# althonos/pyfastani

Measured on AMD Instinct MI355X. Metric: genome-pair ANI/sec (5 Mb bacterial, 3 kb frags), higher is better.
Workload: dtype u32

## Files before the change

### include/fastani_hip.h

```cpp
#ifndef FASTANI_HIP_H
#define FASTANI_HIP_H

#include <stdint.h>

#ifdef __cplusplus
extern "C" {
#endif

#define FA_OK 0
#define FA_ERR_INVALID 1
#define FA_ERR_NO_DEVICE 2
#define FA_ERR_NOMEM 3
#define FA_ERR_UNSUPPORTED 4
#define FA_ERR_INTERNAL 5
#define FA_ERR_IO 6
#define FA_ERR_BUFFER 7

typedef struct fa_sketch fa_sketch;
typedef struct fa_mapper fa_mapper;
typedef struct fa_genomes fa_genomes;

typedef struct fa_params {
  int32_t kmer_size;
  int32_t window_size;
// ... 119 lines not shown

int fa_mapper_debug_mappings(fa_mapper *m, fa_mapping *out, int64_t cap, int64_t *n);
int fa_mapper_debug_l1(fa_mapper *m, int32_t *frag, int32_t *seq_id, int32_t *range_start, int32_t *range_end,
                       int64_t cap, int64_t *n);
int fa_mapper_debug_query_sketch(fa_mapper *m, int64_t fragment, uint32_t *hashes, int32_t cap, int32_t *sketch_size);
int fa_debug_sketch_sequence(const fa_params *params, const void *data, int64_t length, int char_width,
                             uint32_t *hash, int32_t *wpos, int64_t cap, int64_t *n);

int fa_debug_probe_occupancy(int lds_bytes, int *peak_alive);
int fa_mapper_debug_items(fa_mapper *m, void *out, int64_t bytes);
int fa_mapper_debug_links(fa_mapper *m, int32_t *prev, int32_t *fwd, int32_t *bwd, uint8_t *flags, int64_t cap, int64_t *n);
int fa_mapper_debug_locus_events(fa_mapper *m, uint32_t *events, int64_t cap, int64_t *n);
int fa_mapper_last_timings(fa_mapper *m, float *ms, int n);
int fa_mapper_debug_spec(fa_mapper *m, int64_t *out, int n);
int fa_mapper_set_stage_events(fa_mapper *m, int on);
int fa_mapper_stream(fa_mapper *m, void **stream);
int fa_bench_sketch_kernel(fa_mapper *m, fa_genomes *g, int repeat, float *ms_per_launch, uint64_t *bases,
                           uint64_t *minimizers);

#ifdef __cplusplus
}
#endif
#endif
```

### pyfastani_amd/_lib.py

```python
import ctypes as C
import os

_HERE = os.path.dirname(os.path.abspath(__file__))
LIB_PATH = os.path.join(_HERE, "lib", "libfastani_hip.so")

FA_OK, FA_ERR_INVALID, FA_ERR_NO_DEVICE, FA_ERR_NOMEM, FA_ERR_UNSUPPORTED, FA_ERR_INTERNAL, FA_ERR_IO, FA_ERR_BUFFER = range(8)


class Params(C.Structure):
    _fields_ = [
        ("kmer_size", C.c_int32),
        ("window_size", C.c_int32),
        ("fragment_length", C.c_int32),
        ("alphabet_size", C.c_int32),
        ("min_fraction", C.c_float),
        ("percentage_identity", C.c_float),
        ("p_value", C.c_double),
        ("reference_size", C.c_uint64),
    ]


class CgiRow(C.Structure):
    _fields_ = [
        ("query_id", C.c_int32),
# ... 88 lines not shown
    "fa_packed_append": (_i32, [_vp, _P(C.c_char_p), _i32]),
    "fa_packed_free": (None, [_vp]),
    "fa_packed_info": (_i32, [_vp, _P(_i32), _P(C.c_uint64), _P(_i64), _P(_i64)]),
    "fa_sketch_add_packed": (_i32, [_vp, _vp, _i32, _i32, _P(_i64), _P(_i64)]),
    "fa_genomes_reload_packed": (_i32, [_vp, _vp, _vp, _i32, _i32]),
    "fa_genomes_reload_fasta": (_i32, [_vp, _vp, _P(C.c_char_p), _i32]),
    "fa_sketch_add_genomes": (_i32, [_vp, _P(_vp), _P(_i64), _P(_i32), _i64, _i32, _i32, _P(_i32)]),
    "fa_sketch_add_fasta_many": (_i32, [_vp, _P(C.c_char_p), _i32, _P(_i64), _P(_i64)]),
    "fa_debug_probe_occupancy": (_i32, [_i32, _P(_i32)]),
    "fa_mapper_debug_items": (_i32, [_vp, _vp, _i64]),
    "fa_mapper_debug_locus_events": (_i32, [_vp, _vp, _i64, _vp]),
    "fa_mapper_debug_links": (_i32, [_vp, _vp, _vp, _vp, _vp, _i64, _vp]),
    "fa_mapper_last_timings": (_i32, [_vp, _P(_f32), _i32]),
    "fa_mapper_debug_spec": (_i32, [_vp, _P(_i64), _i32]),
    "fa_mapper_set_stage_events": (_i32, [_vp, _i32]),
    "fa_mapper_stream": (_i32, [_vp, _P(_vp)]),
    "fa_bench_sketch_kernel": (_i32, [_vp, _vp, _i32, _P(_f32), _P(_u64), _P(_u64)]),
}

if not os.path.exists(LIB_PATH):
    raise ImportError(
        f"{LIB_PATH} is missing: build it with `python -c 'import __graft_entry__ as g; g.build()'` "
        "(hipcc --offload-arch=gfx950). pyfastani_amd has no CPU fallback."
    )



os.environ.setdefault("GPU_MAX_HW_QUEUES", "8")
lib = C.CDLL(LIB_PATH)
for _name, (_res, _args) in SIGNATURES.items():
# ... 32 lines not shown
```

### pyfastani_amd/csrc/fa_engine.hip

```cpp
#include <cstring>

#include <rocprim/rocprim.hpp>

#include <algorithm>
#include <atomic>
#include <chrono>
#include <climits>
#include <cstdlib>
#include <cstring>
#include <memory>
#include <condition_variable>
#include <mutex>
#include <shared_mutex>
#include <string>
#include <utility>
#include <vector>
#include <cstddef>
#include <deque>

#include "fa_common.h"
#include "fa_fasta.h"
#include "fa_lease.h"
#include "fa_map.hip.h"
#include "fa_policy.h"
// ... 395 lines not shown
  DevBuf<int32_t> map_chunk_count;
  DevBuf<int64_t> map_chunk_off;
  DevBuf<fa_hit_mapping> maps_dev;
  const int32_t *lut_min_hits = nullptr, *lut_pass = nullptr;
  const float *lut_ident = nullptr;
  int64_t last_F = 0;
  uint32_t last_loci = 0;
  uint32_t loci_n = 1, loci_shift = 0;
  uint32_t last_region_count[LOCI_REGIONS] = {0};
  uint64_t last_items = 0;
  const fa_genomes *last_genomes = nullptr;
  float last_ms[MS_SLOTS] = {0};
  hipEvent_t ev[6] = {nullptr};
  int64_t pass_F = 0;
  Forms forms, last_forms;
  std::unique_ptr<fa_genomes> query_batch;
  PinnedBuf pin_image, pin_rows;
  ~Workspace() {
    for (auto &e : ev) if (e) (void)hipEventDestroy(e);
    if (stream) (void)hipStreamDestroy(stream);
    if (h_status) (void)hipHostFree(h_status);
  }
};

struct fa_mapper {
  fa_params P;
  int device = -1;
  hipStream_t stream = nullptr;
  std::mutex mtx;
  DevBuf<uint32_t> rec_hash, uniq_hash, uniq_off, pos_ridx;
// ... 8 lines not shown
  bool events_packed() const { return packed_geo && !env_set("FA_NO_PACKED_GEO"); }
  int64_t N = 0, U = 0;
  int32_t C = 0, G = 0, table_bits = 4, freq_threshold = INT_MAX, total_bins = 0;
  std::vector<uint64_t> lengths;
  std::vector<int32_t> seqs_by_file;
  int32_t cmw = 0, qcap = 1;
  StatTables stats;
  DevBuf<int32_t> d_min_hits, d_pass;
  DevBuf<float> d_ident;
  Spec spec;
  static constexpr int NWS = 4;
  Workspace ws[NWS];
  std::condition_variable ws_free;
  int last_ws = 0;
  bool stage_events = false;
  std::vector<DevBuf<int32_t>> retired_i32;
  std::vector<DevBuf<float>> retired_f32;

  IndexView view() const {
    IndexView v;
    v.rec_hash = rec_hash.p; v.rec_seq = rec_seq.p; v.rec_wpos = rec_wpos.p; v.rec_prev = rec_prev.p; v.rec_fwd = rec_fwd.p; v.rec_bwd = rec_bwd.p; v.rec_flags = rec_flags.p;
    v.rec_hg = packed_geo ? rec_hg.p : nullptr; v.rec_prev16 = packed_geo ? rec_prev16.p : nullptr; v.rec_gpos = rec_gpos.p; v.wrap_rec = wrap_rec.p; v.n_wraps = n_wraps; v.gpos_bits = gpos_bits;
    v.uniq_hash = uniq_hash.p; v.uniq_off = uniq_off.p; v.pos_ridx = pos_ridx.p; v.table = table.p;
    v.contig_rec = contig_rec.p; v.contig_genome = contig_genome.p; v.contig_bin = contig_bin.p; v.genome_bin = genome_bin.p;
    v.N = N; v.U = U; v.C = C; v.G = G; v.table_bits = table_bits; v.freq_threshold = freq_threshold; v.total_bins = total_bins;
    return v;
  }
};

__global__ void k_contig_bins(const int32_t *contig_rec, const int32_t *rec_wpos, int C, int bin_len, int32_t *nbins) {
// ... 373 lines not shown
    ea.chunk_count = w.map_chunk_count.p; ea.chunk_off = w.map_chunk_off.p;
    ea.maps = maps.dev + maps.base; ea.cap = maps.cap - maps.base; ea.total_maps = &w.status.p->total_maps;
    if (map_chunks) hipLaunchKernelGGL(k_map_count, dim3(map_chunks), dim3(256), 0, st, ea);
    hipLaunchKernelGGL(k_map_scan, dim3(1), dim3(1024), 0, st, ea);
    if (map_chunks) hipLaunchKernelGGL(k_map_write, dim3(map_chunks), dim3(256), 0, st, ea);
  }
  struct Part {
    const Spec &sp;
    const int64_t f0, f1, F;
    const int t0, ntiles;
    const int smax;
    const int64_t l_cap;
    L1Plan l1;
    bool scan_sorted = false;
    bool wide = false;
    LociRegions loci{nullptr, 1, 0};
    const int32_t *frag_order = nullptr;
    uint32_t order_len = 0;
    Part(QueryPass &q, Run &r)
        : sp(r.sp), f0(r.f0), f1(r.f1), F(r.f1 - r.f0), t0(q.g.frag_tile_lo[r.f0]),
          ntiles(q.g.frag_tile_lo[r.f1] - q.g.frag_tile_lo[r.f0]), smax(r.sp.smax),
          l_cap(std::max<int64_t>(r.sp.l_cap, (int64_t)std::min<uint32_t>(LOCI_REGIONS, ev_regions_for(r.f1 - r.f0)))) {}
  };

  void launch_part(Run &r) {
    Part p(*this, r);
    const Spec &sp = p.sp;
    const int64_t f0 = p.f0, F = p.F;
    w.last_F = 0; w.last_loci = 0;
    const int ntiles = p.ntiles;
// ... 12 lines not shown
    const int64_t l_cap = p.l_cap;
    {
      static const L1Knobs knobs{(int)env_num("FA_L1_PREFILTER", -1), (float)env_num("FA_L1_THIN_SMALL", -1.0), (float)env_num("FA_L1_THIN_MID", 0.05)};
      p.l1 = plan_l1(sp, m.N, knobs);
      static const bool dbg_l1 = env_set("FA_DEBUG_L1");
      if (dbg_l1) fprintf(stderr, "k_l1 classes: need=%u tiny=%.3f small=%.3f mid=%.3f prefilter=%d -> %d launch(es)\n", p.l1.need, sp.l1_tiny_share, sp.l1_small_share, sp.l1_mid_share, (int)p.l1.prefilter, p.l1.n);
    }
    w.l_frag.ensure((size_t)l_cap); w.l_seq.ensure((size_t)l_cap); w.l_start.ensure((size_t)l_cap); w.l_end.ensure((size_t)l_cap + 4);
    w.l_rfirst.ensure((size_t)l_cap); w.l_rlast.ensure((size_t)l_cap + 4); w.l_rpart.ensure((size_t)l_cap);
    w.l_group.ensure((size_t)l_cap); w.l_shared.ensure((size_t)l_cap); w.l_pos.ensure((size_t)l_cap);
    w.group_best.ensure((size_t)l_cap + 2);
    w.l_beg.ensure((size_t)l_cap); w.l_end0.ensure((size_t)l_cap); w.l_last.ensure((size_t)l_cap); w.l_ndrop.ensure((size_t)l_cap);
    w.l_nev.ensure((size_t)l_cap); w.l_ioff.ensure((size_t)l_cap); w.l_redo.ensure((size_t)l_cap + 4);
    static const int scan_order_knob = (int)env_num("FA_L2_SCAN_ORDER", -1);
    p.scan_sorted = scan_sorted(sp, scan_order_knob);
    w.scan_hist.ensure((size_t)2 * LOCI_REGIONS * SCAN_CLASSES);
    if (p.scan_sorted) w.scan_order.ensure((size_t)l_cap + 64);
    w.ovf_buf.ensure((size_t)sp.scratch_words + 4);
    p.loci.count = w.status.p->loci_region;
    p.loci.n = std::min<uint32_t>(LOCI_REGIONS, ev_regions_for(F));
    p.loci.shift = (uint32_t)floor_log2((int)std::max<int64_t>(1, l_cap / p.loci.n));
    w.loci_n = p.loci.n; w.loci_shift = p.loci.shift;
    p.wide = wide_events(smax);
    w.items.ensure(((size_t)sp.items_cap + 8) * (p.wide ? 4 : 2));
    w.forms = Forms();
    w.forms.n_l1 = p.l1.n;
    for (int c = 0; c < p.l1.n; c++) w.forms.l1_threads[c] = p.l1.c[c].nt;
    w.forms.prefilter = p.l1.prefilter; w.forms.scan_sorted = p.scan_sorted; w.forms.wide = p.wide; w.forms.redo = sp.redo;
    w.forms.smax = smax; w.forms.seed_slots = p.l1.seed_slots();

    launch_sketch_stage(r, p);
    prepare_order(p);
    launch_l1_stage(p);
    launch_l2_stage(r, p);
    launch_cgi_stage_and_hand_over(r, p);
  }

  void prepare_order(Part &p) {
    static const bool order_on = env_num("FA_FRAG_ORDER", 1) != 0;
    static const bool order_one = env_num("FA_FRAG_ORDER_ONE", 1) != 0;
    if (!frag_order_gate(order_on, order_one, NQ, p.F)) return;
    if (w.order_batch != g.serial || w.order_f0 != p.f0 || w.order_f1 != p.f1) {
      std::vector<int32_t> ord;
// ... 125 lines not shown
      a.items = w.items.p; a.items_cap = sp.items_cap; a.pinfo = d_pinfo; a.l_cap = (int32_t)l_cap;
      a.l_shared = w.l_shared.p; a.l_pos = w.l_pos.p; a.pass_lut = w.lut_pass; a.group_best = w.group_best.p;
      a.counters = d_counters; a.loci = p.loci; a.qcap = qcap; a.cmw = m.cmw;
      a.cnt_slots = smax + 1;
      a.rec_total = (unsigned long long *)&d_totals[TOT_RECORDS];
      a.ev_region = w.status.p->ev_region; a.rec_region = w.status.p->rec_region;
      a.n_regions = ev_regions_for(F);
      a.region_cap = (sp.items_cap / a.n_regions) & ~7ULL;
      a.l_redo = w.l_redo.p;
      a.redo_count = &d_counters[CNT_WIDE];
      const L2Lds lds(m.P, smax, wide);
      a.scan_class_div = p.scan_sorted ? lds.scan_class_div : 0;
      a.scan_hist = w.scan_hist.p; a.scan_cursor = w.scan_hist.p + LOCI_REGIONS * SCAN_CLASSES;
      a.scan_order = p.scan_sorted ? w.scan_order.p : nullptr;
      a.f_loci_lo = w.f_loci_lo.p; a.f_loci_n = w.f_loci_n.p;
      a.frag_order = p.frag_order;
      const uint32_t ev_grid = p.frag_order ? p.order_len : (uint32_t)F;
      if (p.frag_order) r.ordered = true;
      a.ev_stage = lds.ev_stage;
      const size_t ev_lds = lds.events;
      FA_REQUIRE(ev_lds <= 150 * 1024, FA_ERR_UNSUPPORTED, "query sketch too large for the LDS-staged event kernel");
      auto pick_lanes = [&](int bytes) {
        int ln = L2_THREADS;
        while (ln > 1 && lds.scan(ln, bytes) > 144 * 1024) ln >>= 1;
        FA_REQUIRE(lds.scan(ln, bytes) <= 160 * 1024, FA_ERR_UNSUPPORTED, "query sketch too large for the LDS-resident L2 state");
        return ln;
      };
      const int lanes8 = pick_lanes(1), lanes16 = pick_lanes(2);
      const size_t lds8 = lds.scan(lanes8, 1), lds16 = lds.scan(lanes16, 2);
      auto scan_grid = [&](int lanes) { return (unsigned)(p.loci.n * (uint32_t)ceil_div((int64_t)1 << p.loci.shift, lanes)); };
      auto launch = [&](auto ev_kernel, auto scan8, auto scan8_rt, auto scan16, auto scan16_rt) {
        launch_lds(ev_kernel, dim3(ev_grid), dim3(EV_THREADS), ev_lds, st, a);
        debug_sync(st, "l2 events");
        if (p.scan_sorted)
          hipLaunchKernelGGL(k_l2_order, dim3((unsigned)(p.loci.n * (uint32_t)ceil_div((int64_t)1 << p.loci.shift, 256))), dim3(256), 0, st, a);
        a.lanes = lanes8;
        launch_lds(lanes8 == L2_THREADS ? scan8 : scan8_rt, dim3(scan_grid(lanes8)), dim3(L2_THREADS), lds8, st, a);
        if (!sp.redo) return;
        a.lanes = lanes16;
        launch_lds(lanes16 == L2_THREADS ? scan16 : scan16_rt, dim3(scan_grid(lanes16)), dim3(L2_THREADS), lds16, st, a);
      };
      const bool pk = m.events_packed();
      if (wide) launch(pk ? k_l2_events<uint32_t, true> : k_l2_events<uint32_t, false>, k_l2_scan<uint32_t, uint8_t, 64>, k_l2_scan<uint32_t, uint8_t, 0>, k_l2_scan<uint32_t, uint16_t, 64>, k_l2_scan<uint32_t, uint16_t, 0>);
      else launch(pk ? k_l2_events<uint16_t, true> : k_l2_events<uint16_t, false>, k_l2_scan<uint16_t, uint8_t, 64>, k_l2_scan<uint16_t, uint8_t, 0>, k_l2_scan<uint16_t, uint16_t, 64>, k_l2_scan<uint16_t, uint16_t, 0>);
    }
    debug_sync(st, "l2 scan");
    if (m.stage_events) FA_HIP(hipEventRecord(w.ev[3], st));
  }

  void launch_cgi_stage_and_hand_over(Run &r, Part &p) {
    const Spec &sp = p.sp;
    const int64_t f0 = p.f0;
    const int64_t l_cap = p.l_cap;
    uint32_t *const d_counters = w.status.p->counters;
    if (npairs > 0) {
      CgiArgs a;
      a.stamp = &w.status.p->stamp[3];
      a.ix = ix; a.group_best = w.group_best.p; a.counters = d_counters; a.l_frag = w.l_frag.p; a.l_seq = w.l_seq.p;
      a.l_pos = w.l_pos.p; a.q_size = w.q_size.p; a.ident_lut = w.lut_ident;
// ... 49 lines not shown
      w.last_ms[MS_L2_EVENTS] += ev_ms;
    }
    const unsigned long long *stamp = h.stamp;
    for (int i = 0; i < 4; i++) w.last_ms[MS_STAGE + i] += (float)((double)(stamp[i + 1] - stamp[i]) * 1e-5);
    t_begin = std::min(t_begin, stamp[0]); t_end = std::max(t_end, stamp[4]);
    w.last_F = F;
    w.last_loci = (uint32_t)v.loci;
    for (uint32_t i = 0; i < LOCI_REGIONS; i++)
      w.last_region_count[i] = i < w.loci_n ? (uint32_t)std::min<uint64_t>(h.loci_region[i], 1ULL << w.loci_shift) : 0u;
    w.last_items = v.events;
    const uint32_t *c = h.counters;
    w.last_ms[MS_RECORDS] += (float)v.records;
    w.last_ms[MS_LOCI] += (float)v.loci;
    w.last_ms[MS_EVENTS] += (float)v.events;
    w.last_ms[MS_WIDE] += (float)c[CNT_WIDE];
    w.last_ms[MS_L1_SORTED] += (float)c[CNT_L1_SORTED]; w.last_ms[MS_L1_MERGED] += (float)c[CNT_L1_MERGED];
    w.last_ms[MS_L1_OFF_FAST] += (float)(c[CNT_MERGED] + c[CNT_OFF_FAST]);
    if (c[CNT_L1_SORTED] + c[CNT_L1_MERGED] > 0) {
      const double nf = (double)(c[CNT_L1_SORTED] + c[CNT_L1_MERGED]);
      fprintf(stderr, "[fa] k_l1 phases, shader-clock ticks per fragment (thread 0):");
      for (int i = 0; i < 8; i++) fprintf(stderr, " %.0f", (double)h.dbg[i] / nf);
      fprintf(stderr, "  (%u block-sorted, %u merged; one workgroup in 64 sampled; gave up on probes / blocks / counts: %llu %llu %llu; expansion: bitmaps+places %.0f, pairs+bitmaps %.0f, bits %.0f)\n",
              c[CNT_L1_SORTED], c[CNT_L1_MERGED], h.dbg[8], h.dbg[9], h.dbg[10], (double)h.dbg[11] / nf, (double)h.dbg[12] / nf, (double)h.dbg[13] / nf);
    }
    return true;
  }


  int64_t run() {
    w.last_F = 0; w.last_loci = 0; w.last_genomes = &g;
// ... 45 lines not shown
    *maps.count = maps.base + pass.nmaps;
    FA_REQUIRE(pass.nmaps <= maps.cap - maps.base, FA_ERR_INVALID, "mapping buffer too small");
    maps.base += pass.nmaps;
  }
  return nrows;
}

struct MapRequest { fa_hit_mapping *maps; int64_t cap; int64_t *n_maps; bool device; };

static int64_t run_query(fa_mapper &m, Workspace &w, const fa_genomes &g, int32_t first, int32_t count, fa_cgi_row *rows, int64_t cap, bool rows_device,
                         const MapRequest *want = nullptr) {
  require_device();
  FA_REQUIRE(first >= 0 && count >= 0 && first + count <= g.n_genomes, FA_ERR_INVALID, "genome range out of bounds");
  for (float &x : w.last_ms) x = 0;
  w.last_forms = Forms();
  fa_cgi_row *dst = rows;
  if (!rows_device) { w.rows_dev.ensure((size_t)std::max<int64_t>(cap, 1)); dst = w.rows_dev.p; }
  const bool one_pass = count > 0 && g.genome_frag_lo[first + count] - g.genome_frag_lo[first] <= pass_fragments();
  fa_cgi_row *host_rows = nullptr;
  if (!rows_device && one_pass && cap <= 65536) {
    w.pin_rows.ensure(std::max<size_t>((size_t)cap * sizeof(fa_cgi_row), 4096));
    FA_HIP(hipHostGetDevicePointer((void **)&host_rows, w.pin_rows.p, 0));
  }
  MapSink sink;
  if (want) {
    FA_REQUIRE(want->cap >= 0 && (want->maps || want->cap == 0) && want->n_maps, FA_ERR_INVALID, "mapping buffer missing");
    sink.on = true; sink.cap = want->cap; sink.dev = want->maps; sink.count = want->n_maps;
    if (!want->device) { w.maps_dev.ensure((size_t)std::max<int64_t>(want->cap, 1)); sink.dev = w.maps_dev.p; }
    *want->n_maps = 0;
  }
// ... 967 lines not shown
      for_each_locus_slice(w, [&](size_t first, size_t count) {
        const size_t c = (size_t)std::max<int64_t>(0, std::min<int64_t>((int64_t)count, cap - k));
        if (c) FA_HIP(hipMemcpyAsync(events + k, w.l_nev.p + first, c * 4, hipMemcpyDeviceToHost, w.stream));
        k += (int64_t)count;
      });
      FA_HIP(hipStreamSynchronize(w.stream));
    }
    *n = k;
  });
}
int fa_mapper_set_stage_events(fa_mapper *m, int on) {
  std::lock_guard<std::mutex> lock(m->mtx);
  m->stage_events = on != 0;
  return FA_OK;
}
int fa_mapper_last_timings(fa_mapper *m, float *ms, int n) {
  std::lock_guard<std::mutex> lock(m->mtx);
  for (int i = 0; i < n && i < MS_SLOTS; i++) ms[i] = m->ws[m->last_ws].last_ms[i];
  return FA_OK;
}
int fa_mapper_debug_spec(fa_mapper *m, int64_t *out, int n) {
  std::lock_guard<std::mutex> lock(m->mtx);
  const Spec &s = m->spec;
  const Forms &f = m->ws[m->last_ws].last_forms;
  auto ppm = [](float share) { return (int64_t)std::lround((double)share * 1e6); };
  const int64_t v[] = {s.init, s.smax, s.seed_slots, ppm(s.l1_small_share), ppm(s.l1_mid_share), ppm(s.l1_tiny_share),
                       s.l1_prefilter, s.l1_no_small, s.l2_loci_last, s.redo, s.part_frags, s.fuse_skip, s.fuse_penalty,
                       s.smax_misses, (int64_t)s.scratch_words, (int64_t)s.items_cap, s.l_cap,
                       f.n_l1, f.l1_threads[0], f.l1_threads[1], f.l1_threads[2], f.prefilter, f.scan_sorted, f.wide, f.fused,
                       f.ordered, f.redo, f.smax, f.seed_slots};
  for (int i = 0; i < n; i++) out[i] = i < (int)(sizeof(v) / sizeof(v[0])) ? v[i] : 0;
  return FA_OK;
}
int fa_mapper_stream(fa_mapper *m, void **stream) { *stream = (void *)m->stream; return FA_OK; }

int fa_bench_sketch_kernel(fa_mapper *m, fa_genomes *g, int repeat, float *ms_per_launch, uint64_t *bases, uint64_t *minimizers) {
  return guarded([&] {
    WorkspaceLease lease(*m);
    Workspace &w = *lease.w;
    require_device();
    int ntiles = (int)g->ntiles;
    FA_REQUIRE(ntiles > 0 && repeat > 0, FA_ERR_INVALID, "nothing to sketch");
    const Tile *tiles = g->tiles;
    DevBuf<Tile> retiled;
    const int tile_len = k1_tile_len(m->P.window_size);
// ... 53 lines not shown
```

### pyfastani_amd/csrc/fa_map.hip.h

```cpp
#pragma once

#include "fa_common.h"
#include "fa_policy.h"
#include "fa_sketch.hip.h"
#include "fa_sketch_fast.hip.h"

namespace fa {



constexpr int MAP_THREADS = 256;
constexpr uint32_t SEED_PAD = 0xFFFFFFFFu;

__device__ inline void block_bitonic_sort(uint32_t *a, uint32_t n32) {
  for (uint32_t size = 2; size <= n32; size <<= 1) {
    for (uint32_t stride = size >> 1; stride > 0; stride >>= 1) {
      __syncthreads();
      for (uint32_t t = threadIdx.x; t < n32 / 2; t += blockDim.x) {
        uint32_t lo = 2 * t - (t & (stride - 1));
        uint32_t hi = lo + stride;
        bool up = (lo & size) == 0;
        uint32_t x = a[lo], y = a[hi];
        if ((x > y) == up) { a[lo] = y; a[hi] = x; }
      }
// ... 1620 lines not shown
  int32_t cnt_slots;
  int32_t lanes;
  int32_t ev_stage;
  unsigned long long *rec_total;
  unsigned long long *ev_region, *rec_region;
  uint64_t region_cap;
  uint32_t n_regions;
  uint8_t *l_redo;
  uint32_t *redo_count;
  const uint32_t *f_loci_lo, *f_loci_n;
  const int32_t *frag_order;
  unsigned long long *stamp;
  uint32_t *scan_hist, *scan_cursor;
  uint32_t *scan_order;
  int32_t scan_class_div;
};

constexpr int L2_THREADS = 64;
constexpr int EV_THREADS = 256;
constexpr int SCAN_CLASSES = 32;
__device__ __forceinline__ uint32_t scan_class(uint32_t nev, int32_t div) {
  return (uint32_t)(SCAN_CLASSES - 1) - min((uint32_t)(SCAN_CLASSES - 1), nev / (uint32_t)div);
}

template <typename T> struct EvBits;
template <> struct EvBits<uint16_t> { static constexpr int RANK = EV_RANK16; };
template <> struct EvBits<uint32_t> { static constexpr int RANK = 24; };
constexpr int EV_DM = 0, EV_DW = 2, EV_DROP = 5, EV_SLOT = 6;
template <typename T> constexpr uint32_t ev_noeval() { return 1u << (8 * sizeof(T) - 1); }
template <typename T> constexpr uint32_t ev_slot_mask() { return ((1u << EvBits<T>::RANK) - 1u) << EV_SLOT; }
// ... 274 lines not shown
  int lbase, LNB, s;
  int rl, g, shared, best, beg, opt_s, opt_e;
  uint32_t overflow;

  static __device__ __forceinline__ uint32_t ld(int addr) { return (uint32_t)*(lds_ptr)(uintptr_t)(uint32_t)addr; }
  static __device__ __forceinline__ void sto(int addr, uint32_t v) { *(lds_ptr)(uintptr_t)(uint32_t)addr = (ST)v; }

  __device__ __forceinline__ void init(ST *st, int lane, int lanes, int sketch, int beg0) {
    lbase = (int)(uint32_t)(uintptr_t)(lds_ptr)st + lane * STB;
    LNB = (LNT ? LNT : lanes) * STB;
    s = sketch;
    rl = lbase; g = 0; shared = 0; best = -1; beg = opt_s = opt_e = beg0; overflow = 0;
  }
  static constexpr uint32_t EMPTY = 2u;
  __device__ __forceinline__ void clear() { for (int i = 0; i <= s + 1; i++) sto(i * LNB + lbase, EMPTY); }
  template <int SH> __device__ __forceinline__ int slot_addr(uint32_t word) const {
    if constexpr (LNT == 64) {
      const uint32_t row = (SH ? word >> SH : word) & ev_slot_mask<T>();
      if constexpr (BASE0) return (int)((STB == 1 ? row : row * STB) | (uint32_t)lbase);
      else return (int)(STB == 1 ? row : row * STB) + lbase;
    } else {
      return (int)__builtin_amdgcn_ubfe(word, SH + EV_SLOT, RB) * LNB + lbase;
    }
  }
  template <int SH> __device__ __forceinline__ void fill(uint32_t word) {
    const int dM = __builtin_amdgcn_sbfe(word, SH + EV_DM, 2), dW = __builtin_amdgcn_sbfe(word, SH + EV_DW, 2);
    const int addr = slot_addr<SH>(word);
    const uint32_t nv = (ld(addr) + (uint32_t)(dW << 1)) ^ ((uint32_t)dM & 1u);
    overflow |= nv;
    sto(addr, nv);
  }
  __device__ __forceinline__ void read_pivot() {
    int rstar = s, F = s, acc = 0, m_acc = 0;
    bool hit = false;
    for (int r = 0; r < s; r++) {
      const uint32_t v = ld((r + 1) * LNB + lbase);
      const int c = (int)(v >> 1) - 1, mt = (int)(v & 1u);
      const bool now = !hit && r + acc + c >= s;
      rstar = now ? r : rstar;
      F = now ? r + acc : F;
      shared = now ? m_acc : shared;
      hit = hit || now;
      acc += c; m_acc += mt;
    }
    F = hit ? F : s + acc;
    shared = hit ? shared : m_acc;
    g = F - s;
    rl = rstar * LNB + lbase;
    best = shared;
  }
  template <int SH> __device__ __forceinline__ void step(uint32_t word) {
    const int dM = __builtin_amdgcn_sbfe(word, SH + EV_DM, 2), dW = __builtin_amdgcn_sbfe(word, SH + EV_DW, 2);
    const int drp = (int)__builtin_amdgcn_ubfe(word, SH + EV_DROP, 1);
    const int addr = slot_addr<SH>(word);
    const int addrb = rl + drp * LNB;
    const uint32_t v = ld(addr), vb0 = ld(addrb);
    const uint32_t nv = (v + (uint32_t)(dW << 1)) ^ ((uint32_t)dM & 1u);
    overflow |= nv;
    sto(addr, nv);
    const bool below = addr <= rl;
    const int dWb = below ? dW : 0;
    shared += below ? dM : 0;
    g += dWb;
    const uint32_t vb = (addrb == addr) ? nv : vb0;
// ... 22 lines not shown
  if (threadIdx.x < SCAN_CLASSES) sh_cnt[threadIdx.x] = 0;
  __syncthreads();
  const uint32_t l = (r << a.loci.shift) + off;
  uint32_t c = 0, rank = 0;
  if (off < live) { c = scan_class(a.l_nev[l], a.scan_class_div); rank = atomicAdd(&sh_cnt[c], 1u); }
  __syncthreads();
  if (threadIdx.x < SCAN_CLASSES) {
    uint32_t before = 0;
    for (uint32_t q = 0; q < threadIdx.x; q++) before += a.scan_hist[r * SCAN_CLASSES + q];
    sh_at[threadIdx.x] = before + (sh_cnt[threadIdx.x] ? atomicAdd(&a.scan_cursor[r * SCAN_CLASSES + threadIdx.x], sh_cnt[threadIdx.x]) : 0u);
  }
  __syncthreads();
  if (off < live) a.scan_order[(r << a.loci.shift) + min(sh_at[c] + rank, (1u << a.loci.shift) - 1u)] = l;
}

template <typename T, typename ST, int LNT>
__global__ __launch_bounds__(L2_THREADS) void k_l2_scan(L2Args a) {
  extern __shared__ __align__(16) unsigned char lds[];
  constexpr bool REDO = sizeof(ST) > 1;
  const int LN = LNT ? LNT : a.lanes;
  ST *st = (ST *)lds;
  const int lane = threadIdx.x;
  if (lane >= LN) return;
  const uint32_t region = blockIdx.x & (a.loci.n - 1u), off = (blockIdx.x / a.loci.n) * (uint32_t)LN + (uint32_t)lane;
  if (a.counters[CNT_LOCI_OVF] || off >= (1u << a.loci.shift) || off >= a.loci.count[region]) return;
  if (a.scan_order && a.pinfo[PI_FLAGS]) return;
  const uint32_t l = a.scan_order ? a.scan_order[(region << a.loci.shift) + off] : (region << a.loci.shift) + off;
  if (REDO) { if (!a.l_redo[l]) return; }
  else a.l_redo[l] = 0;
  const int s = a.q_size[a.l_frag[l]];
  if (s + 1 > a.cnt_slots) return;
  const int beg0 = a.l_beg[l];
  const uint32_t nev = a.l_nev[l];
  constexpr int PER = 16 / sizeof(T);
  const uint4 *ev = (const uint4 *)((const T *)a.items + a.l_ioff[l]);
  Slide<T, ST, LNT, true> sl;
  sl.init(st, lane, LN, s, beg0);
  sl.clear();
  if (sl.lbase != lane * (int)sizeof(ST)) __builtin_trap();

  const uint32_t ngroups = nev / PER;
  const uint32_t fill_groups = min(ngroups, (uint32_t)((((a.l_end0[l] - beg0) + 7) & ~7) / PER));
  auto word_of = [](const uint4 &g, int q) __attribute__((always_inline)) {
    constexpr int WPE = (int)sizeof(T);
    return (q * WPE / 4 == 0) ? g.x : (q * WPE / 4 == 1) ? g.y : (q * WPE / 4 == 2) ? g.z : g.w;
  };
  uint4 cur = ngroups ? ev[0] : make_uint4(0, 0, 0, 0);
  for (uint32_t g = 0; g < fill_groups; g++) {
    const uint4 nxt = (g + 1 < ngroups) ? ev[g + 1] : make_uint4(0, 0, 0, 0);
#pragma unroll
    for (int q = 0; q < PER; q++) {
      if (sizeof(T) == 2 && (q & 1)) sl.template fill<16>(word_of(cur, q)); else sl.template fill<0>(word_of(cur, q));
    }
    cur = nxt;
  }
  sl.read_pivot();
  if (!fill_groups) sl.best = -1;
  for (uint32_t g = fill_groups; g < ngroups; g++) {
    const uint4 nxt = (g + 1 < ngroups) ? ev[g + 1] : make_uint4(0, 0, 0, 0);
#pragma unroll
    for (int q = 0; q < PER; q++) {
      if (sizeof(T) == 2 && (q & 1)) sl.template step<16>(word_of(cur, q)); else sl.template step<0>(word_of(cur, q));
    }
    cur = nxt;
  }
  if (sl.overflow >> Slide<T, ST, LNT, true>::SBITS) {
    if (!REDO) { a.l_redo[l] = 1; atomicAdd(a.redo_count, 1u); return; }
  }
  a.l_shared[l] = sl.best < 0 ? 0 : sl.best;
  a.l_pos[l] = (a.ix.rec_wpos[sl.opt_s] + a.ix.rec_wpos[sl.opt_e]) / 2;
  if (sl.best >= a.pass_lut[s]) {
    unsigned long long key = ((unsigned long long)(uint32_t)sl.best << 32) | (unsigned long long)(0xFFFFFFFFu - l);
    atomicMax(&a.group_best[a.l_group[l]], key);
  }
}

struct CgiArgs {
  IndexView ix;
  const unsigned long long *group_best;
// ... 304 lines not shown
```

### pyfastani_amd/csrc/fa_policy.h

```cpp
#pragma once

#include <algorithm>
#include <cstddef>
#include <cstdint>
#include <vector>

#include "fa_error.h"

namespace fa {

constexpr int L1_STAGE = 128;
constexpr uint32_t L1_SMALL_HITS = 16u * 256u, L1_MID_HITS = 16u * 512u - 256u;
constexpr int L1_INPLACE_MAX = 32;
constexpr int LOCI_REGIONS = 64;
constexpr int EV_REGIONS = 64;
constexpr int EV_RANK16 = 9;

constexpr uint32_t SPEC_SMAX = 1, SPEC_SCRATCH = 2, SPEC_LOCI = 4, SPEC_EVENTS = 8, SPEC_QFUSE = 16;
constexpr uint32_t SPEC_LAST = SPEC_QFUSE;
constexpr uint32_t SPEC_VOID = SPEC_SMAX | SPEC_SCRATCH | SPEC_LOCI | SPEC_EVENTS | SPEC_QFUSE;
static_assert(SPEC_VOID == 2 * SPEC_LAST - 1, "every SPEC_* flag voids the part (k_l2_order / k_l2_scan rely on it)");

enum StatSlot : int {
  STAT_SMAX = 0,
  STAT_SMALL, STAT_MID, STAT_TINY,
};
enum TotalSlot : int {
  TOT_SEEDS = 0,
  TOT_MAX_FRAG,
  TOT_SCRATCH,
  TOT_RECORDS,
};
enum CounterSlot : int {
  CNT_MERGED = 0,
  CNT_OFF_FAST,
  CNT_LOCI_OVF,
  CNT_WIDE,
  CNT_ROWS_DONE,
  CNT_L1_SORTED, CNT_L1_MERGED,
};
enum PinfoSlot : int {
  PI_EVENTS = 0,
  PI_FLAGS,
};

struct PassStatus {
  int32_t stats[4];
  int32_t total_rows, pad0;
  int64_t total_maps;
  uint64_t totals[4];
  uint32_t counters[8];
  unsigned long long pinfo[4];
  unsigned long long ev_region[EV_REGIONS], rec_region[EV_REGIONS];
  uint32_t loci_region[LOCI_REGIONS];
  unsigned long long dbg[16];
  unsigned long long stamp[6];
  uint32_t seq, pad1;
};
// ... 105 lines not shown
  }
  const size_t longest = *std::max_element(len, len + 8);
  if ((double)longest * 8.0 > 1.15 * (double)F) return 0;
  out.assign(longest * 8, -1);
  size_t at[8] = {0};
  for (int32_t p = 0; p <= max_off; p++) {
    const size_t x = xcd_of[(size_t)p];
    for (int32_t i = start[(size_t)p]; i < start[(size_t)p + 1]; i++) out[(at[x]++) * 8 + x] = sorted[(size_t)i];
  }
  return (uint32_t)out.size();
}

struct Forms {
  int n_l1 = 0, l1_threads[3] = {0, 0, 0};
  bool prefilter = false, scan_sorted = false, wide = false, fused = false, ordered = false, redo = false;
  int smax = 0;
  uint32_t seed_slots = 0;
  bool small_class() const { return n_l1 > 1 && l1_threads[0] == 256; }
};

struct L1Class { int nt; uint32_t slots, n_lo, n_hi; };
struct L1Plan {
  L1Class c[3];
  int n = 0;
  bool prefilter = false;
  uint32_t need = 0;
  uint32_t seed_slots() const { return c[n - 1].slots; }
};
struct L1Knobs { int prefilter = -1; float thin_small = -1.0f, thin_mid = 0.05f; };

// ... 17 lines not shown
                                      : (sp.l1_tiny_share < 0.0f || sp.l1_tiny_share >= 0.5f);
    const bool keep_m = !keep_s || p.n == 2 || sp.l1_mid_share < 0.0f || sp.l1_mid_share >= k.thin_mid;
    L1Class c[3];
    int n = 0;
    uint32_t lo = 0u;
    if (keep_s) { c[n++] = p.c[0]; lo = p.c[0].n_hi + 1u; }
    if (keep_m) { c[n] = p.c[1]; c[n].n_lo = lo; lo = p.c[1].n_hi == 0xFFFFFFFFu ? lo : p.c[1].n_hi + 1u; n++; }
    if (p.n == 3) { c[n] = p.c[2]; c[n].n_lo = lo; n++; }
    for (int i = 0; i < n; i++) p.c[i] = c[i];
    p.n = n;
  }
  return p;
}

inline bool scan_sorted(const Spec &sp, int knob) { return knob_or(knob, sp.l2_loci_last >= 1024 * 64); }

inline bool l1_near(int64_t records, int knob) { return knob_or(knob, records >= 300000000LL); }

inline bool wide_events(int smax) { return smax + 1 >= (1 << EV_RANK16); }

inline bool frag_order_gate(bool on, bool one, int genomes, int64_t F) { return on && (genomes >= 2 || one) && F >= 64; }

struct Verdict {
  enum Kind { ACCEPTED, VOIDED, SHRUNK, FAILED } kind = ACCEPTED;
  const char *what = nullptr;
  bool miss = false;
  bool fuse_overflow = false;
  uint64_t loci = 0, events = 0, records = 0;
};

// ... 80 lines not shown
```

Measured before the change: 204,400.

## Add optional banded L2 scan with verification fallback and wave-wide LDS clear

Adds an optional banded mode to the L2 sliding-window scan. A prepass computes per-segment running maxima of the event deltas, and the scan only runs the full step logic in the band that can reach a threshold derived from the peak. Events outside the band only update the fill state. If the band result fails verification, the lane rescans the full range. Separately, the LDS window clear now uses a wave-wide 16-byte vector store when the whole wavefront is active, replacing the per-lane scalar loop. The band mode is off by default behind a knob and adds a prepass read of events plus possible rescans.

```diff
diff --git a/include/fastani_hip.h b/include/fastani_hip.h
--- a/include/fastani_hip.h
+++ b/include/fastani_hip.h
@@ -157,6 +157,7 @@
 int fa_mapper_last_timings(fa_mapper *m, float *ms, int n);
 int fa_mapper_debug_spec(fa_mapper *m, int64_t *out, int n);
 int fa_mapper_set_stage_events(fa_mapper *m, int on);
+int fa_mapper_set_l2_band(fa_mapper *m, int form, float scale, int stats);
 int fa_mapper_stream(fa_mapper *m, void **stream);
 int fa_bench_sketch_kernel(fa_mapper *m, fa_genomes *g, int repeat, float *ms_per_launch, uint64_t *bases,
                            uint64_t *minimizers);
diff --git a/pyfastani_amd/_lib.py b/pyfastani_amd/_lib.py
--- a/pyfastani_amd/_lib.py
+++ b/pyfastani_amd/_lib.py
@@ -126,6 +126,7 @@
     "fa_mapper_last_timings": (_i32, [_vp, _P(_f32), _i32]),
     "fa_mapper_debug_spec": (_i32, [_vp, _P(_i64), _i32]),
     "fa_mapper_set_stage_events": (_i32, [_vp, _i32]),
+    "fa_mapper_set_l2_band": (_i32, [_vp, _i32, _f32, _i32]),
     "fa_mapper_stream": (_i32, [_vp, _P(_vp)]),
     "fa_bench_sketch_kernel": (_i32, [_vp, _vp, _i32, _P(_f32), _P(_u64), _P(_u64)]),
 }
diff --git a/pyfastani_amd/csrc/fa_engine.hip b/pyfastani_amd/csrc/fa_engine.hip
--- a/pyfastani_amd/csrc/fa_engine.hip
+++ b/pyfastani_amd/csrc/fa_engine.hip
@@ -433,6 +433,7 @@
   hipEvent_t ev[6] = {nullptr};
   int64_t pass_F = 0;
   Forms forms, last_forms;
+  uint64_t band_fallbacks = 0, band_stepped = 0;
   std::unique_ptr<fa_genomes> query_batch;
   PinnedBuf pin_image, pin_rows;
   ~Workspace() {
@@ -471,6 +472,9 @@
   std::condition_variable ws_free;
   int last_ws = 0;
   bool stage_events = false;
+  int band_knob = -1;
+  float band_scale = -1.0f;
+  bool band_stats = false;
   std::vector<DevBuf<int32_t>> retired_i32;
   std::vector<DevBuf<float>> retired_f32;
 
@@ -874,6 +878,7 @@
     L1Plan l1;
     bool scan_sorted = false;
     bool wide = false;
+    bool band = false;
     LociRegions loci{nullptr, 1, 0};
     const int32_t *frag_order = nullptr;
     uint32_t order_len = 0;
@@ -916,6 +921,8 @@
     w.l_nev.ensure((size_t)l_cap); w.l_ioff.ensure((size_t)l_cap); w.l_redo.ensure((size_t)l_cap + 4);
     static const int scan_order_knob = (int)env_num("FA_L2_SCAN_ORDER", -1);
     p.scan_sorted = scan_sorted(sp, scan_order_knob);
+    static const int band_knob = (int)env_num("FA_L2_BAND", -1);
+    p.band = l2_band(m.band_knob >= 0 ? m.band_knob : band_knob);
     w.scan_hist.ensure((size_t)2 * LOCI_REGIONS * SCAN_CLASSES);
     if (p.scan_sorted) w.scan_order.ensure((size_t)l_cap + 64);
     w.ovf_buf.ensure((size_t)sp.scratch_words + 4);
@@ -929,6 +936,7 @@
     w.forms.n_l1 = p.l1.n;
     for (int c = 0; c < p.l1.n; c++) w.forms.l1_threads[c] = p.l1.c[c].nt;
     w.forms.prefilter = p.l1.prefilter; w.forms.scan_sorted = p.scan_sorted; w.forms.wide = p.wide; w.forms.redo = sp.redo;
+    w.forms.band = p.band;
     w.forms.smax = smax; w.forms.seed_slots = p.l1.seed_slots();
 
     launch_sketch_stage(r, p);
@@ -1084,6 +1092,14 @@
       a.scan_hist = w.scan_hist.p; a.scan_cursor = w.scan_hist.p + LOCI_REGIONS * SCAN_CLASSES;
       a.scan_order = p.scan_sorted ? w.scan_order.p : nullptr;
       a.f_loci_lo = w.f_loci_lo.p; a.f_loci_n = w.f_loci_n.p;
+      static const bool band_uniform = env_num("FA_L2_BAND_UNIFORM", 0) != 0, wave_clear = env_num("FA_L2_WAVE_CLEAR", 1) != 0;
+      static const float band_scale = (float)env_num("FA_L2_BAND_SCALE", BAND_SCALE);
+      static const bool band_stats = env_num("FA_L2_BAND_STATS", 0) != 0;
+      a.band = p.band ? (band_uniform ? 2 : 1) : 0;
+      a.band_scale = m.band_scale >= 0.0f ? m.band_scale : band_scale;
+      a.band_stats = (band_stats || m.band_stats) ? 1 : 0;
+      a.wave_clear = wave_clear ? 1 : 0;
+      a.band_fallbacks = &d_counters[CNT_BAND_FALLBACK]; a.band_stepped = &d_pinfo[PI_BAND_STEPPED];
       a.frag_order = p.frag_order;
       const uint32_t ev_grid = p.frag_order ? p.order_len : (uint32_t)F;
       if (p.frag_order) r.ordered = true;
@@ -1111,8 +1127,13 @@
         launch_lds(lanes16 == L2_THREADS ? scan16 : scan16_rt, dim3(scan_grid(lanes16)), dim3(L2_THREADS), lds16, st, a);
       };
       const bool pk = m.events_packed();
-      if (wide) launch(pk ? k_l2_events<uint32_t, true> : k_l2_events<uint32_t, false>, k_l2_scan<uint32_t, uint8_t, 64>, k_l2_scan<uint32_t, uint8_t, 0>, k_l2_scan<uint32_t, uint16_t, 64>, k_l2_scan<uint32_t, uint16_t, 0>);
-      else launch(pk ? k_l2_events<uint16_t, true> : k_l2_events<uint16_t, false>, k_l2_scan<uint16_t, uint8_t, 64>, k_l2_scan<uint16_t, uint8_t, 0>, k_l2_scan<uint16_t, uint16_t, 64>, k_l2_scan<uint16_t, uint16_t, 0>);
+      auto launch_form = [&](auto ev_tag, auto band_tag) {
+        typedef decltype(ev_tag) E;
+        constexpr bool B = decltype(band_tag)::value;
+        launch(pk ? k_l2_events<E, true> : k_l2_events<E, false>, k_l2_scan<E, uint8_t, 64, B>, k_l2_scan<E, uint8_t, 0, B>, k_l2_scan<E, uint16_t, 64, B>, k_l2_scan<E, uint16_t, 0, B>);
+      };
+      if (wide) { if (a.band) launch_form(uint32_t(), std::true_type()); else launch_form(uint32_t(), std::false_type()); }
+      else { if (a.band) launch_form(uint16_t(), std::true_type()); else launch_form(uint16_t(), std::false_type()); }
     }
     debug_sync(st, "l2 scan");
     if (m.stage_events) FA_HIP(hipEventRecord(w.ev[3], st));
@@ -1192,6 +1213,7 @@
     w.last_ms[MS_LOCI] += (float)v.loci;
     w.last_ms[MS_EVENTS] += (float)v.events;
     w.last_ms[MS_WIDE] += (float)c[CNT_WIDE];
+    w.band_fallbacks += c[CNT_BAND_FALLBACK]; w.band_stepped += h.pinfo[PI_BAND_STEPPED];
     w.last_ms[MS_L1_SORTED] += (float)c[CNT_L1_SORTED]; w.last_ms[MS_L1_MERGED] += (float)c[CNT_L1_MERGED];
     w.last_ms[MS_L1_OFF_FAST] += (float)(c[CNT_MERGED] + c[CNT_OFF_FAST]);
     if (c[CNT_L1_SORTED] + c[CNT_L1_MERGED] > 0) {
@@ -1267,6 +1289,7 @@
   FA_REQUIRE(first >= 0 && count >= 0 && first + count <= g.n_genomes, FA_ERR_INVALID, "genome range out of bounds");
   for (float &x : w.last_ms) x = 0;
   w.last_forms = Forms();
+  w.band_fallbacks = 0; w.band_stepped = 0;
   fa_cgi_row *dst = rows;
   if (!rows_device) { w.rows_dev.ensure((size_t)std::max<int64_t>(cap, 1)); dst = w.rows_dev.p; }
   const bool one_pass = count > 0 && g.genome_frag_lo[first + count] - g.genome_frag_lo[first] <= pass_fragments();
@@ -2264,6 +2287,13 @@
   m->stage_events = on != 0;
   return FA_OK;
 }
+int fa_mapper_set_l2_band(fa_mapper *m, int form, float scale, int stats) {
+  std::lock_guard<std::mutex> lock(m->mtx);
+  m->band_knob = form < 0 ? -1 : (form != 0);
+  m->band_scale = scale < 0.0f ? -1.0f : scale;
+  m->band_stats = stats != 0;
+  return FA_OK;
+}
 int fa_mapper_last_timings(fa_mapper *m, float *ms, int n) {
   std::lock_guard<std::mutex> lock(m->mtx);
   for (int i = 0; i < n && i < MS_SLOTS; i++) ms[i] = m->ws[m->last_ws].last_ms[i];
@@ -2272,13 +2302,14 @@
 int fa_mapper_debug_spec(fa_mapper *m, int64_t *out, int n) {
   std::lock_guard<std::mutex> lock(m->mtx);
   const Spec &s = m->spec;
-  const Forms &f = m->ws[m->last_ws].last_forms;
+  const Workspace &w = m->ws[m->last_ws];
+  const Forms &f = w.last_forms;
   auto ppm = [](float share) { return (int64_t)std::lround((double)share * 1e6); };
   const int64_t v[] = {s.init, s.smax, s.seed_slots, ppm(s.l1_small_share), ppm(s.l1_mid_share), ppm(s.l1_tiny_share),
                        s.l1_prefilter, s.l1_no_small, s.l2_loci_last, s.redo, s.part_frags, s.fuse_skip, s.fuse_penalty,
                        s.smax_misses, (int64_t)s.scratch_words, (int64_t)s.items_cap, s.l_cap,
                        f.n_l1, f.l1_threads[0], f.l1_threads[1], f.l1_threads[2], f.prefilter, f.scan_sorted, f.wide, f.fused,
-                       f.ordered, f.redo, f.smax, f.seed_slots};
+                       f.ordered, f.redo, f.smax, f.seed_slots, f.band, (int64_t)w.band_fallbacks, (int64_t)w.band_stepped};
   for (int i = 0; i < n; i++) out[i] = i < (int)(sizeof(v) / sizeof(v[0])) ? v[i] : 0;
   return FA_OK;
 }
diff --git a/pyfastani_amd/csrc/fa_map.hip.h b/pyfastani_amd/csrc/fa_map.hip.h
--- a/pyfastani_amd/csrc/fa_map.hip.h
+++ b/pyfastani_amd/csrc/fa_map.hip.h
@@ -1658,6 +1658,12 @@
   uint32_t *scan_hist, *scan_cursor;
   uint32_t *scan_order;
   int32_t scan_class_div;
+  int32_t band;
+  float band_scale;
+  int32_t band_stats;
+  int32_t wave_clear;
+  uint32_t *band_fallbacks;
+  unsigned long long *band_stepped;
 };
 
 constexpr int L2_THREADS = 64;
@@ -1962,6 +1968,15 @@
   }
   static constexpr uint32_t EMPTY = 2u;
   __device__ __forceinline__ void clear() { for (int i = 0; i <= s + 1; i++) sto(i * LNB + lbase, EMPTY); }
+  static __device__ __forceinline__ void clear_wave(int lane, int rows) {
+    typedef uint32_t vec4 __attribute__((ext_vector_type(4)));
+    typedef __attribute__((address_space(3))) vec4 *lds_vec;
+    constexpr uint32_t E = STB == 1 ? EMPTY * 0x01010101u : EMPTY * 0x00010001u;
+    const uint32_t bytes = (uint32_t)rows * 64u * (uint32_t)STB;
+    for (uint32_t o = (uint32_t)lane * 16u; o < bytes; o += 64u * 16u) *(lds_vec)(uintptr_t)o = vec4{E, E, E, E};
+    __builtin_amdgcn_fence(__ATOMIC_ACQ_REL, "wavefront");
+    __builtin_amdgcn_wave_barrier();
+  }
   template <int SH> __device__ __forceinline__ int slot_addr(uint32_t word) const {
     if constexpr (LNT == 64) {
       const uint32_t row = (SH ? word >> SH : word) & ev_slot_mask<T>();
@@ -1978,7 +1993,12 @@
     overflow |= nv;
     sto(addr, nv);
   }
-  __device__ __forceinline__ void read_pivot() {
+  template <int SH> __device__ __forceinline__ void skip(uint32_t word) {
+    fill<SH>(word);
+    beg += (int)__builtin_amdgcn_ubfe(word, SH + EV_DROP, 1);
+  }
+  __device__ __forceinline__ void read_pivot() { read_pivot_state(); best = shared; }
+  __device__ __forceinline__ void read_pivot_state() {
     int rstar = s, F = s, acc = 0, m_acc = 0;
     bool hit = false;
     for (int r = 0; r < s; r++) {
@@ -1995,7 +2015,6 @@
     shared = hit ? shared : m_acc;
     g = F - s;
     rl = rstar * LNB + lbase;
-    best = shared;
   }
   template <int SH> __device__ __forceinline__ void step(uint32_t word) {
     const int dM = __builtin_amdgcn_sbfe(word, SH + EV_DM, 2), dW = __builtin_amdgcn_sbfe(word, SH + EV_DW, 2);
@@ -2048,7 +2067,7 @@
   if (off < live) a.scan_order[(r << a.loci.shift) + min(sh_at[c] + rank, (1u << a.loci.shift) - 1u)] = l;
 }
 
-template <typename T, typename ST, int LNT>
+template <typename T, typename ST, int LNT, bool BAND = false>
 __global__ __launch_bounds__(L2_THREADS) void k_l2_scan(L2Args a) {
   extern __shared__ __align__(16) unsigned char lds[];
   constexpr bool REDO = sizeof(ST) > 1;
@@ -2070,33 +2089,126 @@
   const uint4 *ev = (const uint4 *)((const T *)a.items + a.l_ioff[l]);
   Slide<T, ST, LNT, true> sl;
   sl.init(st, lane, LN, s, beg0);
-  sl.clear();
   if (sl.lbase != lane * (int)sizeof(ST)) __builtin_trap();
 
   const uint32_t ngroups = nev / PER;
-  const uint32_t fill_groups = min(ngroups, (uint32_t)((((a.l_end0[l] - beg0) + 7) & ~7) / PER));
+  const int n_win = a.l_end0[l] - beg0;
+  const uint32_t fill_groups = min(ngroups, (uint32_t)(((n_win + 7) & ~7) / PER));
   auto word_of = [](const uint4 &g, int q) __attribute__((always_inline)) {
     constexpr int WPE = (int)sizeof(T);
     return (q * WPE / 4 == 0) ? g.x : (q * WPE / 4 == 1) ? g.y : (q * WPE / 4 == 2) ? g.z : g.w;
   };
-  uint4 cur = ngroups ? ev[0] : make_uint4(0, 0, 0, 0);
-  for (uint32_t g = 0; g < fill_groups; g++) {
-    const uint4 nxt = (g + 1 < ngroups) ? ev[g + 1] : make_uint4(0, 0, 0, 0);
-#pragma unroll
-    for (int q = 0; q < PER; q++) {
-      if (sizeof(T) == 2 && (q & 1)) sl.template fill<16>(word_of(cur, q)); else sl.template fill<0>(word_of(cur, q));
-    }
-    cur = nxt;
-  }
-  sl.read_pivot();
-  if (!fill_groups) sl.best = -1;
-  for (uint32_t g = fill_groups; g < ngroups; g++) {
-    const uint4 nxt = (g + 1 < ngroups) ? ev[g + 1] : make_uint4(0, 0, 0, 0);
-#pragma unroll
-    for (int q = 0; q < PER; q++) {
-      if (sizeof(T) == 2 && (q & 1)) sl.template step<16>(word_of(cur, q)); else sl.template step<0>(word_of(cur, q));
-    }
-    cur = nxt;
+  const bool full_wave = LNT == 64 && a.wave_clear && __builtin_amdgcn_ballot_w64(true) == ~0ull;
+  if constexpr (!BAND) {
+    if (full_wave) sl.clear_wave(lane, a.cnt_slots + 1); else sl.clear();
+    uint4 cur = ngroups ? ev[0] : make_uint4(0, 0, 0, 0);
+    for (uint32_t g = 0; g < fill_groups; g++) {
+      const uint4 nxt = (g + 1 < ngroups) ? ev[g + 1] : make_uint4(0, 0, 0, 0);
+#pragma unroll
+      for (int q = 0; q < PER; q++) {
+        if (sizeof(T) == 2 && (q & 1)) sl.template fill<16>(word_of(cur, q)); else sl.template fill<0>(word_of(cur, q));
+      }
+      cur = nxt;
+    }
+    sl.read_pivot();
+    if (!fill_groups) sl.best = -1;
+    for (uint32_t g = fill_groups; g < ngroups; g++) {
+      const uint4 nxt = (g + 1 < ngroups) ? ev[g + 1] : make_uint4(0, 0, 0, 0);
+#pragma unroll
+      for (int q = 0; q < PER; q++) {
+        if (sizeof(T) == 2 && (q & 1)) sl.template step<16>(word_of(cur, q)); else sl.template step<0>(word_of(cur, q));
+      }
+      cur = nxt;
+    }
+    if (a.band_stats) atomicAdd(a.band_stepped, (unsigned long long)((ngroups - fill_groups) * (uint32_t)PER));
+  } else {
+  Band band{fill_groups, ngroups, true};
+  int tau = 0;
+  {
+    constexpr uint32_t GPS = BAND_SG_EVENTS / PER;
+    const uint32_t pre_groups = ngroups <= (uint32_t)BAND_SGS * GPS ? ngroups : 0u;
+    int M = 0, m_peak = 0;
+    auto sg_word = [&](int wi) __attribute__((always_inline)) {
+      uint32_t word = 0;
+      if (!__builtin_amdgcn_ballot_w64((uint32_t)wi * 4u * GPS < pre_groups)) return word;
+#pragma unroll 1
+      for (int k = 0; k < 4; k++) {
+        int mx = 0;
+#pragma unroll 4
+        for (uint32_t j = 0; j < GPS; j++) {
+          const uint32_t g = (uint32_t)(wi * 4 + k) * GPS + j;
+          const uint4 w = g < pre_groups ? ev[g] : make_uint4(0, 0, 0, 0);
+#pragma unroll
+          for (int q = 0; q < PER; q++) {
+            M += __builtin_amdgcn_sbfe(word_of(w, q), ((sizeof(T) == 2 && (q & 1)) ? 16 : 0) + EV_DM, 2);
+            mx = max(mx, M);
+          }
+        }
+        word |= band_pack(mx) << (8 * k);
+        m_peak = max(m_peak, mx);
+      }
+      return word;
+    };
+    static_assert(BAND_WORDS == 5, "the words of maxima are spelt out");
+    const uint32_t packed[BAND_WORDS] = {sg_word(0), sg_word(1), sg_word(2), sg_word(3), sg_word(4)};
+    tau = band_tau(m_peak, n_win, s, a.band_scale);
+    band = band_of(packed, ngroups, fill_groups, PER, tau);
+    if (a.band == 2) {
+      uint32_t lo = 0xFFFFFFFFu, hi = 0u;
+      for (uint64_t live = __builtin_amdgcn_ballot_w64(true); live; live &= live - 1) {
+        const int src = __builtin_ctzll(live);
+        lo = min(lo, (uint32_t)__builtin_amdgcn_readlane((int)band.g0, src));
+        hi = max(hi, (uint32_t)__builtin_amdgcn_readlane((int)band.g1, src));
+      }
+      band.g0 = min(band.g0, max(lo, fill_groups));
+      band.g1 = max(band.g1, min(hi, ngroups));
+      band.whole = band.whole || (band.g0 == fill_groups && band.g1 == ngroups);
+    }
+  }
+
+  uint32_t stepped = 0, fell_back = 0, overflow = 0;
+  bool todo = true;
+#pragma unroll 1
+  for (int round = 0; round < 2; round++) {
+    if (!__builtin_amdgcn_ballot_w64(todo)) break;
+    if (full_wave) sl.clear_wave(lane, a.cnt_slots + 1);
+    else if (todo) sl.clear();
+    const uint32_t g0 = todo ? band.g0 : 0u, g1 = todo ? band.g1 : 0u;
+    if (todo) { overflow |= sl.overflow; sl.init(st, lane, LN, s, beg0); }
+    uint4 cur = g1 ? ev[0] : make_uint4(0, 0, 0, 0);
+    uint32_t g = 0;
+    for (; g < g0; g++) {
+      const uint4 nxt = (g + 1 < ngroups) ? ev[g + 1] : make_uint4(0, 0, 0, 0);
+#pragma unroll
+      for (int q = 0; q < PER; q++) {
+        if (sizeof(T) == 2 && (q & 1)) sl.template skip<16>(word_of(cur, q)); else sl.template skip<0>(word_of(cur, q));
+      }
+      cur = nxt;
+    }
+    if (todo) {
+      sl.read_pivot_state();
+      sl.best = (g0 == fill_groups && fill_groups) ? sl.shared : -1;
+    }
+    for (; g < g1; g++) {
+      const uint4 nxt = (g + 1 < ngroups) ? ev[g + 1] : make_uint4(0, 0, 0, 0);
+#pragma unroll
+      for (int q = 0; q < PER; q++) {
+        if (sizeof(T) == 2 && (q & 1)) sl.template step<16>(word_of(cur, q)); else sl.template step<0>(word_of(cur, q));
+      }
+      cur = nxt;
+    }
+    if (todo) {
+      stepped += (g1 - g0) * (uint32_t)PER;
+      todo = !band_verified(band, sl.best, tau);
+      fell_back += todo ? 1u : 0u;
+      band = Band{fill_groups, ngroups, true};
+    }
+  }
+  if (a.band_stats) {
+    atomicAdd(a.band_stepped, (unsigned long long)stepped);
+    if (fell_back) atomicAdd(a.band_fallbacks, fell_back);
+  }
+  sl.overflow |= overflow;
   }
   if (sl.overflow >> Slide<T, ST, LNT, true>::SBITS) {
     if (!REDO) { a.l_redo[l] = 1; atomicAdd(a.redo_count, 1u); return; }
diff --git a/pyfastani_amd/csrc/fa_policy.h b/pyfastani_amd/csrc/fa_policy.h
--- a/pyfastani_amd/csrc/fa_policy.h
+++ b/pyfastani_amd/csrc/fa_policy.h
@@ -38,10 +38,12 @@
   CNT_WIDE,
   CNT_ROWS_DONE,
   CNT_L1_SORTED, CNT_L1_MERGED,
+  CNT_BAND_FALLBACK,
 };
 enum PinfoSlot : int {
   PI_EVENTS = 0,
   PI_FLAGS,
+  PI_BAND_STEPPED,
 };
 
 struct PassStatus {
@@ -177,6 +179,7 @@
 struct Forms {
   int n_l1 = 0, l1_threads[3] = {0, 0, 0};
   bool prefilter = false, scan_sorted = false, wide = false, fused = false, ordered = false, redo = false;
+  bool band = false;
   int smax = 0;
   uint32_t seed_slots = 0;
   bool small_class() const { return n_l1 > 1 && l1_threads[0] == 256; }
@@ -224,6 +227,60 @@
 }
 
 inline bool scan_sorted(const Spec &sp, int knob) { return knob_or(knob, sp.l2_loci_last >= 1024 * 64); }
+
+#if defined(__HIPCC__)
+#define FA_HD __host__ __device__
+#else
+#define FA_HD
+#endif
+constexpr int BAND_SG_EVENTS = 64;
+constexpr int BAND_SGS = 20;
+constexpr int BAND_WORDS = BAND_SGS / 4;
+constexpr int BAND_M_MAX = 510;
+constexpr float BAND_SCALE = 0.85f;
+static_assert(BAND_SGS % 4 == 0, "the maxima fill whole 32-bit words");
+
+FA_HD inline uint32_t band_pack(int mx) { return (uint32_t)((mx + 1) >> 1); }
+
+constexpr int BAND_TAU_NEVER = 0x7FFFFFFF;
+FA_HD inline int band_tau(int m_peak, int n_win, int s, float c) {
+  if (c > 2.0f) return BAND_TAU_NEVER;
+  const int den = s + n_win - m_peak;
+  if (!(c > 0.0f) || m_peak <= 0 || m_peak > BAND_M_MAX || s <= 0 || den <= 0) return 0;
+  const float k = (float)s * (float)m_peak / (float)den;
+  const float t = c * k;
+  const int tau = t >= (float)m_peak ? m_peak : (int)t;
+  return tau < 0 ? 0 : tau;
+}
+
+struct Band { uint32_t g0, g1; bool whole; };
+FA_HD inline void band_word(uint32_t word, int base, uint32_t nsg, uint32_t tau, int &first, int &last) {
+  for (int k = 0; k < 4; k++) {
+    const uint32_t stored = (word >> (8 * k)) & 0xFFu;
+    const bool in = (uint32_t)(base + k) < nsg && 2u * stored >= tau;
+    first = (in && first < 0) ? base + k : first;
+    last = in ? base + k : last;
+  }
+}
+FA_HD inline Band band_of(const uint32_t (&packed)[BAND_WORDS], uint32_t ngroups, uint32_t fill_groups, int per, int tau) {
+  const uint32_t gps = (uint32_t)(BAND_SG_EVENTS / per);
+  if (tau == BAND_TAU_NEVER) return Band{fill_groups, fill_groups, false};
+  if (tau <= 0 || ngroups > (uint32_t)BAND_SGS * gps) return Band{fill_groups, ngroups, true};
+  const uint32_t nsg = (ngroups + gps - 1u) / gps;
+  int first = -1, last = -1;
+  static_assert(BAND_WORDS == 5, "the words of maxima are spelt out");
+  band_word(packed[0], 0, nsg, (uint32_t)tau, first, last); band_word(packed[1], 4, nsg, (uint32_t)tau, first, last);
+  band_word(packed[2], 8, nsg, (uint32_t)tau, first, last); band_word(packed[3], 12, nsg, (uint32_t)tau, first, last);
+  band_word(packed[4], 16, nsg, (uint32_t)tau, first, last);
+  if (first < 0) return Band{fill_groups, fill_groups, fill_groups == ngroups};
+  const uint32_t lo = (uint32_t)first * gps, hi = (uint32_t)(last + 1) * gps;
+  const uint32_t g0 = lo > fill_groups ? lo : fill_groups, g1c = hi < ngroups ? hi : ngroups, g1 = g1c > g0 ? g1c : g0;
+  return Band{g0, g1, g0 == fill_groups && g1 == ngroups};
+}
+
+FA_HD inline bool band_verified(const Band &b, int best, int tau) { return b.whole || best >= tau; }
+
+inline bool l2_band(int knob) { return knob_or(knob, false); }
 
 inline bool l1_near(int64_t records, int knob) { return knob_or(knob, records >= 300000000LL); }
 
```

Result: no change. 206,300, median of 6 (+0.9%).
